# ychalier/transflow

Hardware: AMD Instinct MI355X
Metric: frames/sec (Farneback+remap) (higher is better)
Workload: dtype f32; 1 GPU; 4k: one clip of T=256 3840x2160 uint8 frames sharded over the ranks (rank r owns pairs shard_range(255, r, 1) + a one-frame halo), Farneback pyr_scale=0.5 levels=5 winsize=15 iterations=3 poly_n=5 poly_sigma=1.2 flags=0, BACKWARD post_process, moveref layer (reset random p=0.5 through a float mask, u drawn on the GPU), 1 RGB pixmap source, render; clip_frames=256, equal_batches=False

## Files before the change

### transflow_amd/csrc/common.h

```cpp
#pragma once
#include <hip/hip_runtime.h>

#include <cstdarg>
#include <cstdint>
#include <cstdio>
#include <cstdlib>
#include <memory>
#include <new>
#include <string>
#include <vector>

#include "../../include/tfhip.h"

#define TF_API extern "C" __attribute__((visibility("default")))

namespace tf {

int set_error(int code, const char *fmt, ...) __attribute__((format(printf, 2, 3)));
hipStream_t stream();
hipStream_t main_stream();
int side_stream(int which, hipStream_t *out);
int ensure_init();

enum Opt { OPT_FB_FUSED = 0, OPT_FB_FUSE_MIN_PX, OPT_FB_NO_SHARE, OPT_FB_NO_OVERLAP, OPT_REMAP_PX, OPT_REMAP_NO_PACK, OPT_REMAP_KEEP_RGBA,
           OPT_PROF_LEVELS, OPT_FB_EXACT_SUMS, OPT_FB_CHAIN, OPT_FB_SEGS, OPT_REMAP_QUAD, OPT_JD_PAR_SUB_BYTES,
           OPT_JD_PAR_GROUP_SUBS, OPT_JD_PAR_STAGED, OPT_REMAP_LEAN, OPT_COUNT };
long option(Opt which);

#ifdef TF_EXPERIMENT
inline long tune(const char *env, long dflt)
{
    const char *v = getenv(env);
    return v ? atol(v) : dflt;
}
inline const char *tune_str(const char *env) { return getenv(env); }
#else
constexpr long tune(const char *, long dflt) { return dflt; }
constexpr const char *tune_str(const char *) { return nullptr; }
#endif

struct StreamScope {
    explicit StreamScope(hipStream_t s);
    ~StreamScope();
    hipStream_t prev;
};

#define TF_HIP(expr)                                                                              \
    do {                                                                                          \
        hipError_t _e = (expr);                                                                   \
        if (_e != hipSuccess)                                                                     \
            return tf::set_error(TF_ERR_HIP, "%s failed: %s (%s:%d)", #expr, hipGetErrorString(_e), \
                                 __FILE__, __LINE__);                                             \
    } while (0)

#define TF_TRY(expr)        \
    do {                    \
        int _rc = (expr);   \
        if (_rc != TF_OK)   \
            return _rc;     \
// ... 110 lines not shown
```

### transflow_amd/csrc/fb_common.h

```cpp
#pragma once
#include <type_traits>
#include <algorithm>
#include <cfloat>
#include <cmath>
#include <cstdlib>
#include <cstring>
#include <map>
#include <memory>
#include <mutex>
#include <string>

#include "common.h"
#include "fb_plan.h"

struct tf_fb;

namespace tf {
namespace fb {

constexpr int MAX_POLY_N = 15;

typedef float float2u __attribute__((ext_vector_type(2), aligned(4)));
typedef float float4u __attribute__((ext_vector_type(4), aligned(4)));

// ... 86 lines not shown
    const unsigned u = (xcd < rn ? xcd * (qn + 1) : rn * (qn + 1) + (xcd - rn) * qn) + (lin >> 3);
    const unsigned whole = u / (S * G);
    unsigned l = 0;
    while (l < 7 && (l + 1) * P / 8 <= whole)
        l++;
    const unsigned p0 = l * P / 8, n = (l + 1) * P / 8 - p0, r = u - p0 * S * G;
    by = r / (S * n);
    const unsigned rem = r - by * S * n;
    bx = rem / n;
    pair = (int)(p0 + (rem - bx * n));
}

__device__ __forceinline__ void lds_barrier()
{
    __builtin_amdgcn_fence(__ATOMIC_RELEASE, "workgroup", "local");
    __builtin_amdgcn_s_barrier();
    __builtin_amdgcn_fence(__ATOMIC_ACQUIRE, "workgroup", "local");
}
__device__ __forceinline__ double fast_recip(double d)
{
    const double r = __builtin_amdgcn_rcp(d);
    return __builtin_fma(__builtin_fma(-d, r, 1.0), r, r);
}

__device__ __forceinline__ void lds_wave_sync()
{
    __builtin_amdgcn_fence(__ATOMIC_RELEASE, "workgroup", "local");
    __builtin_amdgcn_wave_barrier();
    __builtin_amdgcn_fence(__ATOMIC_ACQUIRE, "workgroup", "local");
}

__device__ __forceinline__ int reflect101_once(int p, int len) { return p < 0 ? -p : (p >= len ? 2 * len - 2 - p : p); }
__device__ __forceinline__ int reflect101_near(int p, int len) { return len < 2 ? 0 : reflect101_once(p, len); }

struct ImgTile {
    int TWo, THo;
    int tw_shift;
    int rstride;
    int LW, LH;
    int pitch;
    int same_size;
    double scale_x, scale_y;
};

typedef float f32x2 __attribute__((ext_vector_type(2)));
typedef float f32x4 __attribute__((ext_vector_type(4)));

constexpr int RP_MAX_LEVELS = 4;

__device__ __forceinline__ float border_weight(int d) { return d < 2 ? 0.14f : (d < 5 ? 0.4472f : 1.f); }
__device__ __forceinline__ float border_scale(int x, int y, int W, int H)
{
    const bool fires = (unsigned)(x - 5) >= (unsigned)(W - 10) || (unsigned)(y - 5) >= (unsigned)(H - 10);
    return fires ? border_weight(x) * border_weight(W - x - 1) * border_weight(y) * border_weight(H - y - 1) : 1.f;
}

struct FlowInit {
    int mode;
    const float2 *src;
    int Wc, Hc;
    const int *xofs, *yofs;
    const float *xfrac, *yfrac;
    float mul;
    const int2 *rmap;
};

// ... 113 lines not shown
namespace fb {

inline FlowInit fb_upsampled(tf_fb *fb, int k, const float2 *coarse_flow)
{
    const Level &L = *fb->lv[k], &C = *fb->lv[k + 1];
    FlowInit fi;
    memset(&fi, 0, sizeof(fi));
    fi.mode = 1;
    fi.src = coarse_flow;
    fi.Wc = C.W;
    fi.Hc = C.H;
    fi.xofs = L.flow_lerp.xofs.as<int>();
    fi.yofs = L.flow_lerp.yofs.as<int>();
    fi.xfrac = L.flow_lerp.xfrac.as<float>();
    fi.yfrac = L.flow_lerp.yfrac.as<float>();
    fi.mul = (float)(1. / fb->prm.pyr_scale);
    return fi;
}

inline bool fb_exact(const tf_fb *fb) { return fb->exact >= 0 ? fb->exact != 0 : option(OPT_FB_EXACT_SUMS) != 0; }

struct March {
    int mode, segs, seg;
};

const char *lvl_name(const char *base, int k);

int fb_level_image(tf_fb *fb, int k, const ImageRun &run, bool standalone = false);
bool plan_split_level(int W, int H, Level &L, std::vector<int> &colsrc);
bool plan_quarter_level(int W, int H, const Level &L);
ImgTile choose_tile(int W, int H, int Wk, int Hk, int ksz, int level);
int fb_polyexp(tf_fb *fb, int w, int h, const ImageRun &run, int k = -1);
int fb_expand_level(tf_fb *fb, int k, const ImageRun &run, bool standalone = false);
int fb_m_room(tf_fb *fb, int w, int h, int n_pairs);
int fb_update_matrices(tf_fb *fb, int w, int h, int n_pairs, const FlowInit &fi, int k = -1);
int fb_carry_room(tf_fb *fb, size_t carry_doubles, size_t flags);
int fb_check_fault(tf_fb *fb, const char *where);
int fb_carry_scan(tf_fb *fb, int w, int n_pairs, int segs, int k);
int fb_blur_solve(tf_fb *fb, int w, int h, int n_pairs, float2 *flow_out, int k = -1);
int fb_gauss_solve(tf_fb *fb, int w, int h, int n_pairs, float2 *flow_out, int k = -1);
int fb_setup_flags(tf_fb *fb);
int fb_initial_flow(tf_fb *fb, int n_pairs, float2 *out);
int fb_exact_room(tf_fb *fb, int w, int h, int n_pairs);
int fb_exact_from_matrices(tf_fb *fb, int w, int h, int n_pairs, float2 *flow_out, int k);
int fb_exact_hsolve(tf_fb *fb, int w, int h, int n_pairs, float2 *flow_out, int k);
int fb_w1_solve(tf_fb *fb, int w, int h, int n_pairs, float2 *flow_out);
bool fb_flow_iter_serves(const tf_fb *fb, int w, int h);
int fb_flow_iter(tf_fb *fb, int w, int h, int n_pairs, float2 *flow_out, int k, const FlowInit &fi);

}
}
```

### transflow_amd/csrc/fb_level_image.hip

```cpp
#include "fb_common.h"

namespace {

__device__ __forceinline__ int lerp_coord(int d, double scale, int src, bool zero_at_edges, float &frac)
{
    float f = (float)((d + 0.5) * scale - 0.5);
    int s = (int)floorf(f);
    f -= s;
    if (zero_at_edges) {
        if (s < 0) {
            f = 0.f;
            s = 0;
        }
        if (s >= src - 1) {
            f = 0.f;
            s = src - 1;
        }
    }
    frac = f;
    return s;
}

__global__ void __launch_bounds__(256)
k_level_image(const uint8_t *__restrict__ frames, const int2 *__restrict__ pairs, float *__restrict__ img, int W,
// ... 345 lines not shown
            float *out = L.rowf + (out_row0 + row) * NC + 4 * grp;
            out[0] = acc0.x;
            out[1] = acc1.x;
            if (four) {
                out[2] = acc0.y;
                out[3] = acc1.y;
            }
        }
    }
}

__global__ void __launch_bounds__(RP_THREADS)
k_level_rowpass(const uint8_t *__restrict__ frames, const int2 *__restrict__ pairs, int W, int H, RowPassArgs args, int RB,
                int pitch, int r4, int rmax)
{
    extern __shared__ __attribute__((aligned(16))) uint8_t s_rp[];
    uint8_t *sS = s_rp;
    float *sKall = reinterpret_cast<float *>(s_rp + (size_t)RB * pitch);
    const int pi = blockIdx.y;
    const int2 pr = pairs[pi >> 1];
    const uint8_t *src = frames + (size_t)((pi & 1) ? pr.y : pr.x) * W * H;
    const int y0 = blockIdx.x * RB, nrows = min(RB, H - y0);
    {
        int base = 0;
        for (int l = 0; l < args.n; l++) {
            for (int i = threadIdx.x; i < args.lv[l].ksz; i += RP_THREADS)
                sKall[base + i] = args.lv[l].kern[i];
            base += args.lv[l].ksz;
        }
    }
    const int nq = W >> 2;
    {
        const int lane_ = threadIdx.x & 63, wave_ = threadIdx.x >> 6;
        constexpr int U = 4;
        for (int i = wave_; i < nrows; i += RP_WAVES) {
            const uint32_t *g = reinterpret_cast<const uint32_t *>(src + (size_t)(y0 + i) * W);
            uint32_t *d = reinterpret_cast<uint32_t *>(sS + i * pitch + r4);
            for (int c0 = lane_; c0 < nq; c0 += 64 * U) {
                uint32_t v[U];
#pragma unroll
                for (int u = 0; u < U; u++)
                    if (c0 + 64 * u < nq)
                        v[u] = g[c0 + 64 * u];
#pragma unroll
                for (int u = 0; u < U; u++)
                    if (c0 + 64 * u < nq)
                        d[c0 + 64 * u] = v[u];
            }
        }
    }
    for (int idx = threadIdx.x; idx < nrows * 2 * rmax; idx += RP_THREADS) {
        const int i = idx / (2 * rmax), j = idx - i * 2 * rmax;
        const int c = j < rmax ? j - rmax : W + (j - rmax);
        sS[i * pitch + r4 + c] = src[(size_t)(y0 + i) * W + reflect101(c, W)];
    }
    __syncthreads();
    const int lane = threadIdx.x & 63, wave = threadIdx.x >> 6;
    int kbase = 0;
    for (int l = 0; l < args.n; l++) {
        const RowPassLevel &L = args.lv[l];
        const float *sK = sKall + kbase;
        kbase += L.ksz;
        const size_t out_row0 = (size_t)pi * H + y0;
        if (L.ksz == 9 && L.rshift == 1) {
            rowpass_level_t<9, 1>(L, sS, sK, nrows, pitch, r4, out_row0, lane, wave);
            continue;
        }
        if (L.ksz == 19 && L.rshift == 2) {
            rowpass_level_t<19, 2>(L, sS, sK, nrows, pitch, r4, out_row0, lane, wave);
            continue;
        }
        if (L.ksz == 39 && L.rshift == 3) {
            rowpass_level_t<39, 3>(L, sS, sK, nrows, pitch, r4, out_row0, lane, wave);
            continue;
        }
        if (L.ksz == 79 && L.rshift == 3) {
            rowpass_level_t<79, 3>(L, sS, sK, nrows, pitch, r4, out_row0, lane, wave);
            continue;
        }
        const int ksz = L.ksz, r = ksz >> 1, NC = L.NC, rshift = L.rshift;
        const int R = 1 << rshift, G = 64 >> rshift;
        const int li = lane & (R - 1), lg = lane >> rshift;
        const int ngroups = (NC + 3) >> 2;
        const int n_rb = (nrows + R - 1) >> rshift, n_gb = (ngroups + G - 1) / G;
        for (int item = wave; item < n_rb * n_gb; item += RP_WAVES) {
            const int gb = item % n_gb, rb = item / n_gb;
            const int row = rb * R + li, grp = gb * G + lg;
// ... 161 lines not shown
    const int Wk = W >> 2, Hk = H >> 2;
    unsigned tbx, tby, tbz;
    xcd_tile3(tbx, tby, tbz);
    const int pi = tbz;
    const int2 pr = pairs[pi >> 1];
    const uint8_t *src = frames + (size_t)((pi & 1) ? pr.y : pr.x) * W * H;
    const int X0 = tbx * QI_TW, Y0 = tby * QI_TH;
    const int lane = threadIdx.x & 63, wave = threadIdx.x >> 6;
    const int xs = S * X0 - 4, ys = S * Y0 - 3;
    const bool dwords = xs >= 0 && xs + 4 * PD <= W && ys >= 0 && ys + NR <= H;
    if (dwords) {
        constexpr int U = (NR + 3) / 4;
        for (int j0 = wave; j0 < NR; j0 += 4 * U) {
            uint32_t v[U], v2[U];
#pragma unroll
            for (int u = 0; u < U; u++) {
                const int j = min(j0 + 4 * u, NR - 1);
                const uint32_t *g = reinterpret_cast<const uint32_t *>(src + (size_t)(ys + j) * W + xs);
                v[u] = g[lane];
                v2[u] = g[64 + (lane & 1)];
            }
#pragma unroll
            for (int u = 0; u < U; u++) {
                const int j = j0 + 4 * u;
                if (j < NR) {
                    sS[j * PD + lane] = v[u];
                    if (lane < 2)
                        sS[j * PD + 64 + lane] = v2[u];
                }
            }
        }
    } else {
        uint8_t *s8 = reinterpret_cast<uint8_t *>(sS);
        for (int j = wave; j < NR; j += 4) {
            const uint8_t *g = src + (size_t)reflect101(ys + j, H) * W;
            for (int b = lane; b < 4 * PD; b += 64)
                s8[j * 4 * PD + b] = g[reflect101(xs + b, W)];
        }
    }
    __syncthreads();
    const int X = X0 + lane, Yw = Y0 + SEG * wave;
    if (X >= Wk || Yw >= Hk)
        return;
    float t[K];
#pragma unroll
    for (int i = 0; i < K; i++)
        t[i] = kern[i];
    const float fx = xfrac[X];
    const uint32_t *q = sS + (S * SEG * wave) * PD + lane;
    constexpr int NROWS = S * (SEG - 1) + 2 + 2 * r;
    float c0[NROWS], c1[NROWS];
    auto row_pair = [&](int j) {
        const uint32_t *qa = q + j * PD, *qb = qa + PD;
        const uint32_t a0 = qa[0], a1 = qa[1], a2 = qa[2], b0 = qb[0], b1 = qb[1], b2 = qb[2];
        const uint32_t wa[3] = {__builtin_amdgcn_alignbyte(a1, a0, 1), __builtin_amdgcn_alignbyte(a2, a1, 1), a2 >> 8};
        const uint32_t wb[3] = {__builtin_amdgcn_alignbyte(b1, b0, 1), __builtin_amdgcn_alignbyte(b2, b1, 1), b2 >> 8};
        f32x2 p[K + 1];
#pragma unroll
        for (int i = 0; i <= K; i++)
            p[i] = f32x2{(float)((wa[i >> 2] >> (8 * (i & 3))) & 0xff), (float)((wb[i >> 2] >> (8 * (i & 3))) & 0xff)};
        f32x2 A0 = t[0] * p[0], A1 = t[0] * p[1];
#pragma unroll
        for (int i = 1; i < K; i++) {
            A0 += t[i] * p[i];
            A1 += t[i] * p[i + 1];
        }
        c0[j] = A0.x;
        c0[j + 1] = A0.y;
        c1[j] = A1.x;
        c1[j + 1] = A1.y;
    };
#pragma unroll
    for (int j = 0; j < 6; j += 2)
        row_pair(j);
    float *dst = img + (size_t)pi * Wk * Hk + X;
#pragma unroll
    for (int y = 0; y < SEG; y++) {
        if (Yw + y >= Hk)
            break;
        row_pair(S * y + 6);
        row_pair(S * y + 8);
        const int m = S * y + r;
        float v00 = t[r] * c0[m], v01 = t[r] * c1[m], v10 = t[r] * c0[m + 1], v11 = t[r] * c1[m + 1];
#pragma unroll
        for (int i = 1; i <= r; i++) {
            const float k = t[r + i];
            v00 += k * (c0[m + i] + c0[m - i]);
            v01 += k * (c1[m + i] + c1[m - i]);
            v10 += k * (c0[m + 1 + i] + c0[m + 1 - i]);
            v11 += k * (c1[m + 1 + i] + c1[m + 1 - i]);
        }
        const float fy = yfrac[Yw + y];
        const float h0 = v00 * (1.f - fx) + v01 * fx, h1 = v10 * (1.f - fx) + v11 * fx;
        dst[(size_t)(Yw + y) * Wk] = h0 * (1.f - fy) + h1 * fy;
    }
}

}

namespace tf {
namespace fb {

int fb_level_image(tf_fb *fb, int k, const ImageRun &run, bool standalone)
{
    Level &L = *fb->lv[k];
    if (L.quarter)
        return launch(lvl_name("fb_level_image", k), k_level_quarter_image, dim3(cdiv(L.W, QI_TW), cdiv(L.H, QI_TH), run.n),
                      dim3(256), 0, (const uint8_t *)fb->frames.as<uint8_t>(), fb->image_list(run), fb->imgk(k), fb->W, fb->H,
                      (const float *)L.kern.as<float>(), (const float *)L.img_lerp.xfrac.as<float>(),
                      (const float *)L.img_lerp.yfrac.as<float>());
    if (L.split) {
        if (k == fb->rp_first || standalone) {
            RowPassArgs a;
            memset(&a, 0, sizeof(a));
            size_t taps = 0;
            for (int j = fb->K; j >= 1; j--) {
                Level &S = *fb->lv[j];
                if (!S.split)
                    continue;
                RowPassLevel &rl = a.lv[a.n++];
                rl.rowf = fb->rowf.as<float>() + S.rowf_off;
                rl.colsrc = S.colsrc.as<int>();
                rl.kern = S.kern.as<float>();
                rl.NC = S.NC;
                rl.ksz = S.ksz;
                rl.rshift = S.rp_rshift;
                taps += (size_t)S.ksz;
            }
            const size_t smem_rp = (size_t)fb->rp_RB * fb->rp_pitch + taps * sizeof(float);
            TF_TRY(launch(lvl_name("fb_level_rowpass", -1), k_level_rowpass, dim3(cdiv(fb->H, fb->rp_RB), run.n),
                          dim3(RP_THREADS), smem_rp, (const uint8_t *)fb->frames.as<uint8_t>(),
                          fb->image_list(run), fb->W, fb->H, a, fb->rp_RB, fb->rp_pitch, fb->rp_r4,
                          fb->rp_rmax));
        }
        return launch(lvl_name("fb_level_colpass", k), k_level_colpass, dim3(cdiv(L.W, 64), cdiv(L.H, 4), run.n), dim3(256),
                      (size_t)L.ksz * sizeof(float), (const float *)(fb->rowf.as<float>() + L.rowf_off), fb->imgk(k), fb->W, fb->H,
                      L.W, L.H, L.NC, (const float *)L.kern.as<float>(), L.ksz, (const int *)L.img_lerp.xofs.as<int>(),
                      (const float *)L.img_lerp.xfrac.as<float>(), (const int *)L.img_lerp.yofs.as<int>(),
// ... 139 lines not shown
```

### transflow_amd/csrc/fb_pyramid.hip

```cpp
#include "fb_common.h"

namespace {

#ifndef TF_PX_TH
#define TF_PX_TH 16
#endif
constexpr int PX_TW = 64, PX_TH = TF_PX_TH;

__global__ void k_polyexp(const float *__restrict__ img, float *__restrict__ R, int Wk, int Hk, PolyConst pc)
{
    extern __shared__ float s_mem[];
    const int n = pc.n;
    const int LW = PX_TW + 2 * n;
    const int LH = PX_TH + 2 * n;
    float *sI = s_mem;
    float *sT = s_mem + LH * LW;
    const int pi = blockIdx.z;
    const size_t Nk = (size_t)Wk * Hk;
    const float *src = img + (size_t)pi * Nk;
    const int x0 = blockIdx.x * PX_TW, y0 = blockIdx.y * PX_TH;
    for (int idx = threadIdx.x; idx < LH * LW; idx += blockDim.x) {
        int ry = idx / LW, cx = idx % LW;
        int y = clampi(y0 - n + ry, 0, Hk - 1), x = clampi(x0 - n + cx, 0, Wk - 1);
        sI[idx] = src[(size_t)y * Wk + x];
// ... 48 lines not shown
        r_store_px(dst, Nk, o, v);
    }
}

typedef float float2w __attribute__((ext_vector_type(2), aligned(4)));

template <int N>
__device__ __forceinline__ void polyexp_vertical4(const f32x2 (&v)[4 + 2 * N], const PolyConst &pc, float *T0, float *T1,
                                                  float *T2, int LW)
{
#pragma unroll
    for (int q = 0; q < 4; q++) {
        const f32x2 c = v[q + N];
        f32x2 t0 = c * pc.g[0], t1 = {0.f, 0.f}, t2 = {0.f, 0.f};
#pragma unroll
        for (int k = 1; k <= N; k++) {
            const f32x2 a = v[q + N - k], b = v[q + N + k];
            const f32x2 p = a + b;
            t0 = t0 + pc.g[k] * p;
            t1 = t1 + pc.xg[k] * (b - a);
            t2 = t2 + pc.xxg[k] * p;
        }
        *reinterpret_cast<f32x2 *>(T0 + q * LW) = t0;
        *reinterpret_cast<f32x2 *>(T1 + q * LW) = t1;
        *reinterpret_cast<f32x2 *>(T2 + q * LW) = t2;
    }
}

template <int N>
__global__ void __launch_bounds__(256)
k_polyexp_t(const float *__restrict__ img, float *__restrict__ R, int Wk, int Hk, PolyConst pc)
{
    constexpr int TW = PX_TW, TH = PX_TH, LW = TW + 2 * N, LH = TH + 2 * N;
    __shared__ float sI[LH * LW];
    __shared__ float sT[3][TH][LW];
    const int pi = blockIdx.z;
    const size_t Nk = (size_t)Wk * Hk;
    const float *src = img + (size_t)pi * Nk;
    const int x0 = blockIdx.x * TW, y0 = blockIdx.y * TH;
    for (int idx = threadIdx.x; idx < LH * LW; idx += 256) {
        int ry = idx / LW, cx = idx - ry * LW;
        int y = clampi(y0 - N + ry, 0, Hk - 1), x = clampi(x0 - N + cx, 0, Wk - 1);
        sI[idx] = src[(size_t)y * Wk + x];
    }
    __syncthreads();
    static_assert(LW % 2 == 0, "column pairs");
    for (int idx = threadIdx.x; idx < (TH / 4) * (LW / 2); idx += 256) {
        const int g = idx / (LW / 2), cx = 2 * (idx - g * (LW / 2));
        f32x2 v[4 + 2 * N];
#pragma unroll
        for (int j = 0; j < 4 + 2 * N; j++)
            v[j] = *reinterpret_cast<const f32x2 *>(&sI[(4 * g + j) * LW + cx]);
        polyexp_vertical4<N>(v, pc, &sT[0][4 * g][cx], &sT[1][4 * g][cx], &sT[2][4 * g][cx], LW);
    }
    __syncthreads();
    float *dst = R + (size_t)pi * 5 * Nk;
    for (int idx = threadIdx.x; idx < TH * (TW / 2); idx += 256) {
        const int ty = idx / (TW / 2), cp = idx - ty * (TW / 2);
        const int x = x0 + 2 * cp, y = y0 + ty;
        if (x >= Wk || y >= Hk)
            continue;
        float w0[2 + 2 * N], w1[2 + 2 * N], w2[2 + 2 * N];
#pragma unroll
        for (int j = 0; j < 2 + 2 * N; j++) {
            w0[j] = sT[0][ty][2 * cp + j];
            w1[j] = sT[1][ty][2 * cp + j];
            w2[j] = sT[2][ty][2 * cp + j];
        }
        float out[2][5];
#pragma unroll
        for (int q = 0; q < 2; q++) {
            const float *T0 = w0 + q + N, *T1 = w1 + q + N, *T2 = w2 + q + N;
            float g0 = pc.g[0];
            double b1 = T0[0] * g0, b2 = 0, b3 = T1[0] * g0, b4 = 0, b5 = T2[0] * g0, b6 = 0;
#pragma unroll
            for (int k = 1; k <= N; k++) {
// ... 236 lines not shown
                        *reinterpret_cast<uint32_t *>(sS + ry * SW + 4 * c) = v[u];
                }
            }
        }
    } else {
        for (int c = lane; c < ncols; c += 64) {
            const int x = reflect101_near(xs + c, W);
            for (int j0 = wave; j0 < nrows; j0 += 4 * U) {
                uint8_t v[U];
#pragma unroll
                for (int u = 0; u < U; u++) {
                    int ry = j0 + 4 * u;
                    if (ry < nrows)
                        v[u] = src[(size_t)reflect101_near(rfirst + ry, H) * W + x];
                }
#pragma unroll
                for (int u = 0; u < U; u++) {
                    int ry = j0 + 4 * u;
                    if (ry < nrows)
                        sS[ry * SW + c] = v[u];
                }
            }
        }
    }
    __syncthreads();
    static_assert(LW % 2 == 0 && SW >= 2 * LW + 8, "2 x 2 blocks; a block's three dwords stay inside its staged row");
    for (int idx = threadIdx.x; idx < ((ny + 1) >> 1) * (LW / 2); idx += 256) {
        const int by2 = idx / (LW / 2), ry = 2 * by2, cx = 2 * (idx - by2 * (LW / 2));
        float rp[6][4];
#pragma unroll
        for (int dy = 0; dy < 6; dy++) {
            const uint32_t *q = reinterpret_cast<const uint32_t *>(sS + (2 * ry + dy) * SW + 2 * cx);
            const uint32_t d0 = q[0], d1 = q[1], d2 = q[2];
            const uint32_t lo = __builtin_amdgcn_alignbyte(d1, d0, off), hi = __builtin_amdgcn_alignbyte(d2, d1, off);
            const float b0 = (float)(lo & 0xff), b1 = (float)((lo >> 8) & 0xff), b2 = (float)((lo >> 16) & 0xff),
                        b3 = (float)(lo >> 24), b4 = (float)(hi & 0xff), b5 = (float)((hi >> 8) & 0xff);
            rp[dy][0] = b1 * kc + (b0 + b2) * k1;
            rp[dy][1] = b2 * kc + (b1 + b3) * k1;
            rp[dy][2] = b3 * kc + (b2 + b4) * k1;
            rp[dy][3] = b4 * kc + (b3 + b5) * k1;
        }
#pragma unroll
        for (int a = 0; a < 2; a++) {
            float out[2];
#pragma unroll
            for (int b = 0; b < 2; b++) {
                float v00 = kc * rp[2 * a + 1][2 * b], v01 = kc * rp[2 * a + 1][2 * b + 1];
                float v10 = kc * rp[2 * a + 2][2 * b], v11 = kc * rp[2 * a + 2][2 * b + 1];
                v00 += k1 * (rp[2 * a + 2][2 * b] + rp[2 * a][2 * b]);
                v01 += k1 * (rp[2 * a + 2][2 * b + 1] + rp[2 * a][2 * b + 1]);
                v10 += k1 * (rp[2 * a + 3][2 * b] + rp[2 * a + 1][2 * b]);
                v11 += k1 * (rp[2 * a + 3][2 * b + 1] + rp[2 * a + 1][2 * b + 1]);
                const float h0 = v00 * (1.f - 0.5f) + v01 * 0.5f, h1 = v10 * (1.f - 0.5f) + v11 * 0.5f;
                out[b] = h0 * (1.f - 0.5f) + h1 * 0.5f;
            }
            if (ry + a < ny)
                *reinterpret_cast<f32x2 *>(sI + (ry + a) * LW + cx) = f32x2{out[0], out[1]};
        }
    }
    __syncthreads();
    tile_expansion<N, TW, TH>(sI, sT, x0, y0, xr0, yr0, Wk, Hk, pc, R + (size_t)pi * 5 * Nk, Nk);
}

}

namespace tf {
namespace fb {

int fb_polyexp(tf_fb *fb, int w, int h, const ImageRun &run, int k)
{
    const int n = fb->pc.n;
    dim3 grid(cdiv(w, PX_TW), cdiv(h, PX_TH), run.n);
    if (n == 5)
        return launch(lvl_name("fb_polyexp", k), k_polyexp_t<5>, grid, dim3(256), 0, (const float *)fb->imgk(k),
                      fb->Rk(k, run), w, h, fb->pc);
    if (n == 7)
        return launch(lvl_name("fb_polyexp", k), k_polyexp_t<7>, grid, dim3(256), 0, (const float *)fb->imgk(k),
                      fb->Rk(k, run), w, h, fb->pc);
    size_t smem = ((size_t)(PX_TH + 2 * n) * (PX_TW + 2 * n) + 3 * (size_t)PX_TH * (PX_TW + 2 * n)) * sizeof(float);
    return launch(lvl_name("fb_polyexp_generic", k), k_polyexp, grid, dim3(256), smem,
                  (const float *)fb->imgk(k), fb->Rk(k, run), w, h, fb->pc);
}

static bool fb_can_fuse_level(tf_fb *fb, int k)
{
    static const bool off = tune("TF_FB_NO_A1A2", 0) != 0;
    const Level &L = *fb->lv[k];
    return !off && L.W == fb->W && L.H == fb->H && L.ksz == 3 && (fb->pc.n == 5 || fb->pc.n == 7);
}

static bool fb_can_fuse_half_level(tf_fb *fb, int k)
{
    static const bool off = tune("TF_FB_NO_A1A2", 0) != 0;
    const Level &L = *fb->lv[k];
    return !off && 2 * L.W == fb->W && 2 * L.H == fb->H && L.ksz == 3 && (fb->pc.n == 5 || fb->pc.n == 7);
}

static int fb_level1_polyexp(tf_fb *fb, int k, const ImageRun &run)
{
    Level &L = *fb->lv[k];
    dim3 grid(cdiv(L.W, 64), cdiv(L.H, TF_EXP_TH1), run.n);
    const float kc = L.kern_host[1], k1 = L.kern_host[2];
    if (fb->pc.n == 5)
        return launch(lvl_name("fb_level_polyexp", k), k_level1_polyexp_t<5>, grid, dim3(256), 0,
                      (const uint8_t *)fb->frames.as<uint8_t>(), fb->image_list(run), fb->Rk(k, run), fb->W,
                      fb->H, kc, k1, fb->pc);
    return launch(lvl_name("fb_level_polyexp", k), k_level1_polyexp_t<7>, grid, dim3(256), 0,
                  (const uint8_t *)fb->frames.as<uint8_t>(), fb->image_list(run), fb->Rk(k, run), fb->W, fb->H,
                  kc, k1, fb->pc);
}

static int fb_level0_polyexp(tf_fb *fb, int k, const ImageRun &run)
{
    Level &L = *fb->lv[k];
    dim3 grid(cdiv(L.W, 64), cdiv(L.H, TF_EXP_TH0), run.n);
    const float kc = L.kern_host[1], k1 = L.kern_host[2];
    if (fb->pc.n == 5)
        return launch(lvl_name("fb_level_polyexp", k), k_level0_polyexp_t<5>, grid, dim3(256), 0,
                      (const uint8_t *)fb->frames.as<uint8_t>(), fb->image_list(run), fb->Rk(k, run),
                      L.W, L.H, kc, k1, fb->pc);
    return launch(lvl_name("fb_level_polyexp", k), k_level0_polyexp_t<7>, grid, dim3(256), 0,
                  (const uint8_t *)fb->frames.as<uint8_t>(), fb->image_list(run), fb->Rk(k, run), L.W,
                  L.H, kc, k1, fb->pc);
}

int fb_expand_level(tf_fb *fb, int k, const ImageRun &run, bool standalone)
{
    if (fb_can_fuse_level(fb, k))
        return fb_level0_polyexp(fb, k, run);
    if (fb_can_fuse_half_level(fb, k))
        return fb_level1_polyexp(fb, k, run);
    TF_TRY(fb_level_image(fb, k, run, standalone));
    return fb_polyexp(fb, fb->lv[k]->W, fb->lv[k]->H, run, k);
}

}
}
```

### transflow_amd/csrc/runtime.hip

```cpp
#include <cstring>
#include <map>
#include <mutex>

#include "common.h"

#include <cstdlib>

namespace tf {

static thread_local std::string g_last_error;
static std::mutex g_mu;
static bool g_inited = false;
static int g_device = 0;
static hipStream_t g_stream = nullptr;

int set_error(int code, const char *fmt, ...)
{
    char buf[1024];
    va_list ap;
    va_start(ap, fmt);
    vsnprintf(buf, sizeof(buf), fmt, ap);
    va_end(ap);
    g_last_error = buf;
    return code;
}

struct OptDef {
    const char *name;
    long value, lo, hi;
};
static OptDef g_opts[OPT_COUNT] = {
    {"fb_fused", -1, -1, 1},
    {"fb_fuse_min_px", 4000000, 0, 1l << 40},
    {"fb_no_share", 0, 0, 1},
    {"fb_no_overlap", 0, 0, 1},
    {"remap_px", 4, 1, 4},
    {"remap_no_pack", 0, 0, 2},
    {"remap_keep_rgba", 0, 0, 1},
    {"prof_levels", 0, 0, 1},
    {"fb_exact_sums", 0, 0, 1},
    {"fb_chain", -1, -1, 1},
    {"fb_segs", 0, 0, 64},
    {"remap_quad", 1, 0, 1},
    {"jd_par_sub_bytes", 0, 0, 1024},
    {"jd_par_group_subs", 0, 0, 256},
    {"jd_par_staged", 0, 0, 1},
    {"remap_lean", 1, 0, 1},
};
long option(Opt which) { return g_opts[which].value; }

static thread_local hipStream_t g_override = nullptr;
static thread_local hipStream_t g_thread_main = nullptr;
static hipStream_t g_thread_streams[3] = {nullptr, nullptr, nullptr};

hipStream_t main_stream() { return g_thread_main ? g_thread_main : g_stream; }
hipStream_t stream() { return g_override ? g_override : main_stream(); }

static hipStream_t g_side[5] = {nullptr, nullptr, nullptr, nullptr, nullptr};
int side_stream(int which, hipStream_t *out)
{
    TF_REQUIRE(which >= 0 && which <= 4, "side_stream: bad index");
    TF_TRY(ensure_init());
    std::lock_guard<std::mutex> lk(g_mu);
    if (!g_side[which]) {
        int least = 0, greatest = 0;
        TF_HIP(hipDeviceGetStreamPriorityRange(&least, &greatest));
        TF_HIP(hipStreamCreateWithPriority(&g_side[which], hipStreamNonBlocking, (which == 0 || which >= 3) ? least : greatest));
    }
    *out = g_side[which];
    return TF_OK;
}

StreamScope::StreamScope(hipStream_t s) : prev(g_override) { g_override = s; }
StreamScope::~StreamScope() { g_override = prev; }

static int init_device(int device)
{
    std::lock_guard<std::mutex> lk(g_mu);
    if (g_inited) {
        if (device != g_device)
// ... 446 lines not shown
```

### transflow_amd/roofline.py

```python
from __future__ import annotations

import json
import os

HBM_PEAK_GBS = 8000.0
HBM_COPY_CEILING_GBS = 6290.0

_ROOT = os.path.dirname(os.path.dirname(os.path.abspath(__file__)))


def level_sizes(width: int, height: int, pyr_scale: float, levels: int):
    k, scale = 0, 1.0
    while k < levels:
        scale *= pyr_scale
        if width * scale < 32 or height * scale < 32:
            break
        k += 1
    out = []
    for lvl in range(k + 1):
        s = 1.0
        for _ in range(lvl):
            s *= pyr_scale
        out.append((int(round_half_even(width * s)), int(round_half_even(height * s))))
    return out
# ... 59 lines not shown
            continue
        if name == "fb_level_polyexp" and k >= 2:
            continue
        if name == "fb_polyexp" and k < 2:
            continue
        if name == "fb_flow_iter" and not level_is_fused(n[k], pairs, fused):
            continue
        if name in ("fb_update_matrices", "fb_blur_solve") and level_is_fused(n[k], pairs, fused):
            continue
        if name == "fb_blur_solve":
            mult = iterations
        elif name in ("fb_update_matrices", "fb_flow_iter"):
            total += (iterations - 1) * pairs * (68 if name == "fb_update_matrices" else 96) * n[k]
        total += mult * kernel_bytes(name, n[0], n[k], nc, pairs)
    return total


def built_kernel_bytes(name, width, height, levels, pairs, iterations=3, fused=-1) -> int:
    n, sizes = _levels(width, height, levels)
    frames = pairs + 1
    total = 0
    if name.startswith("remap_step"):
        return 0
    for k in range(len(n)):
        nc = n[k + 1] if k + 1 < len(n) else 0
        is_fused = level_is_fused(n[k], pairs, fused)
        if name == "fb_flow_iter" and is_fused:
            first = 48 * n[k] + (8 * nc if nc else 0)
            total += pairs * (first + (iterations - 1) * 56 * n[k])
        elif name == "fb_update_matrices" and not is_fused:
            total += pairs * (60 * n[k] + (8 * nc if nc else 0) + (iterations - 1) * 68 * n[k])
        elif name == "fb_blur_solve" and not is_fused:
            total += pairs * iterations * 28 * n[k]
        elif name == "fb_level_polyexp" and k < 2:
            total += frames * (n[0] + 20 * n[k])
        elif name == "fb_level_rowpass" and k >= 2:
            if k == 2:
                total += frames * n[0]
            total += frames * 8 * sizes[0][1] * sizes[k][0]
        elif name == "fb_level_colpass" and k >= 2:
            total += frames * (8 * sizes[0][1] * sizes[k][0] + 4 * n[k])
        elif name == "fb_polyexp" and k >= 2:
            total += frames * 24 * n[k]
    return total


def built_flow_iter_level_bytes(width, height, levels, pairs, iterations=3, fused=-1) -> dict:
    n, _ = _levels(width, height, levels)
    out = {}
    for k in range(len(n)):
        nc = n[k + 1] if k + 1 < len(n) else 0
        if level_is_fused(n[k], pairs, fused):
            out[k] = pairs * (48 * n[k] + (8 * nc if nc else 0) + (iterations - 1) * 56 * n[k])
    return out


BUILT_FB_KERNELS = ("fb_flow_iter", "fb_update_matrices", "fb_blur_solve", "fb_level_polyexp", "fb_level_rowpass",
                    "fb_level_colpass", "fb_polyexp")


def built_remap_bytes(width, height, reset_mask=False, forward=False) -> int:
    state = 8 if width <= 8192 and height <= 8192 else 16
    per_px = (4 + 16 if forward else 8) + state + 3 + 4 + 3 + (4 if reset_mask else 0)
    return per_px * width * height


def built_step_bytes(width, height, levels, pairs, iterations=3, reset_mask=False, forward=False, fused=-1) -> int:
    fb = sum(built_kernel_bytes(k, width, height, levels, pairs, iterations, fused) for k in BUILT_FB_KERNELS)
    rm = pairs * built_remap_bytes(width, height, reset_mask, forward)
    if not forward and pairs >= 2:
        rm -= (pairs - 1) * 4 * width * height
    return fb + rm


def profile_traffic(name, width, height, levels, pairs, launches_per_step, iterations=3, fused=-1):
    table = None
    for fname in ("r05_traffic.json", "r04_traffic.json", "r03_traffic.json", "r02_traffic.json", "r01_traffic.json"):
        path = os.path.join(_ROOT, "profiles", fname)
        if os.path.exists(path):
            with open(path) as f:
                t = json.load(f)
            if name in t:
                table = t
                break
    if table is None:
        return None
    n, _ = _levels(width, height, levels)
    per_level_launches = {"fb_update_matrices": iterations, "fb_blur_solve": iterations,
                          "fb_flow_iter": iterations}.get(name, 1)
    if name == "fb_flow_iter":
        n = [v for v in n if level_is_fused(v, pairs, fused)]
# ... 24 lines not shown
```

Before: 2138 frames/s.

## Split fused level-1 polyexp into standalone half-image kernel plus generic polyexp

Adds a default-on option that splits pyramid level 1 out of the fused downsample+polynomial-expansion kernel. A new register-walking half-resolution image kernel reads the uint8 frame directly and writes a float image, and the generic polyexp then runs on that image. Separately, it batches the global-to-LDS staging loads in the row-pass, quarter-image and polyexp tile kernels (more loads in flight, vectorised float2 loads for interior tiles). Splitting adds an intermediate float image round trip through memory, in exchange for dropping the fused kernel's redundant halo recomputation and LDS pressure.

```diff
diff --git a/transflow_amd/csrc/common.h b/transflow_amd/csrc/common.h
--- a/transflow_amd/csrc/common.h
+++ b/transflow_amd/csrc/common.h
@@ -24,7 +24,7 @@
 
 enum Opt { OPT_FB_FUSED = 0, OPT_FB_FUSE_MIN_PX, OPT_FB_NO_SHARE, OPT_FB_NO_OVERLAP, OPT_REMAP_PX, OPT_REMAP_NO_PACK, OPT_REMAP_KEEP_RGBA,
            OPT_PROF_LEVELS, OPT_FB_EXACT_SUMS, OPT_FB_CHAIN, OPT_FB_SEGS, OPT_REMAP_QUAD, OPT_JD_PAR_SUB_BYTES,
-           OPT_JD_PAR_GROUP_SUBS, OPT_JD_PAR_STAGED, OPT_REMAP_LEAN, OPT_COUNT };
+           OPT_JD_PAR_GROUP_SUBS, OPT_JD_PAR_STAGED, OPT_REMAP_LEAN, OPT_FB_LEVEL1_SPLIT, OPT_COUNT };
 long option(Opt which);
 
 #ifdef TF_EXPERIMENT
diff --git a/transflow_amd/csrc/fb_common.h b/transflow_amd/csrc/fb_common.h
--- a/transflow_amd/csrc/fb_common.h
+++ b/transflow_amd/csrc/fb_common.h
@@ -142,6 +142,33 @@
 
 __device__ __forceinline__ int reflect101_once(int p, int len) { return p < 0 ? -p : (p >= len ? 2 * len - 2 - p : p); }
 __device__ __forceinline__ int reflect101_near(int p, int len) { return len < 2 ? 0 : reflect101_once(p, len); }
+
+__device__ __forceinline__ void half_level_row_pass(uint32_t lo, uint32_t hi, float kc, float k1, float rp[4])
+{
+    const float b0 = (float)(lo & 0xff), b1 = (float)((lo >> 8) & 0xff), b2 = (float)((lo >> 16) & 0xff),
+                b3 = (float)(lo >> 24), b4 = (float)(hi & 0xff), b5 = (float)((hi >> 8) & 0xff);
+    rp[0] = b1 * kc + (b0 + b2) * k1;
+    rp[1] = b2 * kc + (b1 + b3) * k1;
+    rp[2] = b3 * kc + (b2 + b4) * k1;
+    rp[3] = b4 * kc + (b3 + b5) * k1;
+}
+__device__ __forceinline__ void half_level_block(const float (&rp)[6][4], float kc, float k1, float out[2][2])
+{
+#pragma unroll
+    for (int a = 0; a < 2; a++) {
+#pragma unroll
+        for (int b = 0; b < 2; b++) {
+            float v00 = kc * rp[2 * a + 1][2 * b], v01 = kc * rp[2 * a + 1][2 * b + 1];
+            float v10 = kc * rp[2 * a + 2][2 * b], v11 = kc * rp[2 * a + 2][2 * b + 1];
+            v00 += k1 * (rp[2 * a + 2][2 * b] + rp[2 * a][2 * b]);
+            v01 += k1 * (rp[2 * a + 2][2 * b + 1] + rp[2 * a][2 * b + 1]);
+            v10 += k1 * (rp[2 * a + 3][2 * b] + rp[2 * a + 1][2 * b]);
+            v11 += k1 * (rp[2 * a + 3][2 * b + 1] + rp[2 * a + 1][2 * b + 1]);
+            const float h0 = v00 * (1.f - 0.5f) + v01 * 0.5f, h1 = v10 * (1.f - 0.5f) + v11 * 0.5f;
+            out[a][b] = h0 * (1.f - 0.5f) + h1 * 0.5f;
+        }
+    }
+}
 
 struct ImgTile {
     int TWo, THo;
@@ -321,6 +348,7 @@
 ImgTile choose_tile(int W, int H, int Wk, int Hk, int ksz, int level);
 int fb_polyexp(tf_fb *fb, int w, int h, const ImageRun &run, int k = -1);
 int fb_expand_level(tf_fb *fb, int k, const ImageRun &run, bool standalone = false);
+bool fb_split_half_level(tf_fb *fb, int k);
 int fb_m_room(tf_fb *fb, int w, int h, int n_pairs);
 int fb_update_matrices(tf_fb *fb, int w, int h, int n_pairs, const FlowInit &fi, int k = -1);
 int fb_carry_room(tf_fb *fb, size_t carry_doubles, size_t flags);
diff --git a/transflow_amd/csrc/fb_level_image.hip b/transflow_amd/csrc/fb_level_image.hip
--- a/transflow_amd/csrc/fb_level_image.hip
+++ b/transflow_amd/csrc/fb_level_image.hip
@@ -401,27 +401,53 @@
     const int nq = W >> 2;
     {
         const int lane_ = threadIdx.x & 63, wave_ = threadIdx.x >> 6;
-        constexpr int U = 4;
-        for (int i = wave_; i < nrows; i += RP_WAVES) {
+        constexpr int U = 16;
+        for (int i = wave_; i < nrows; i += 2 * RP_WAVES) {
+            const int i2 = i + RP_WAVES;
+            const bool second = i2 < nrows;
             const uint32_t *g = reinterpret_cast<const uint32_t *>(src + (size_t)(y0 + i) * W);
+            const uint32_t *g2 = reinterpret_cast<const uint32_t *>(src + (size_t)(y0 + (second ? i2 : i)) * W);
             uint32_t *d = reinterpret_cast<uint32_t *>(sS + i * pitch + r4);
+            uint32_t *d2 = reinterpret_cast<uint32_t *>(sS + i2 * pitch + r4);
             for (int c0 = lane_; c0 < nq; c0 += 64 * U) {
-                uint32_t v[U];
+                uint32_t v[U], v2[U];
 #pragma unroll
                 for (int u = 0; u < U; u++)
-                    if (c0 + 64 * u < nq)
+                    if (c0 + 64 * u < nq) {
                         v[u] = g[c0 + 64 * u];
+                        v2[u] = g2[c0 + 64 * u];
+                    }
 #pragma unroll
                 for (int u = 0; u < U; u++)
-                    if (c0 + 64 * u < nq)
+                    if (c0 + 64 * u < nq) {
                         d[c0 + 64 * u] = v[u];
-            }
-        }
-    }
-    for (int idx = threadIdx.x; idx < nrows * 2 * rmax; idx += RP_THREADS) {
-        const int i = idx / (2 * rmax), j = idx - i * 2 * rmax;
-        const int c = j < rmax ? j - rmax : W + (j - rmax);
-        sS[i * pitch + r4 + c] = src[(size_t)(y0 + i) * W + reflect101(c, W)];
+                        if (second)
+                            d2[c0 + 64 * u] = v2[u];
+                    }
+            }
+        }
+    }
+    {
+        constexpr int UH = 4;
+        const int nh = nrows * 2 * rmax;
+        for (int idx0 = threadIdx.x; idx0 < nh; idx0 += RP_THREADS * UH) {
+            uint8_t v[UH];
+            int at[UH];
+#pragma unroll
+            for (int u = 0; u < UH; u++) {
+                const int idx = idx0 + RP_THREADS * u;
+                if (idx < nh) {
+                    const int i = idx / (2 * rmax), j = idx - i * 2 * rmax;
+                    const int c = j < rmax ? j - rmax : W + (j - rmax);
+                    at[u] = i * pitch + r4 + c;
+                    v[u] = src[(size_t)(y0 + i) * W + reflect101(c, W)];
+                }
+            }
+#pragma unroll
+            for (int u = 0; u < UH; u++)
+                if (idx0 + RP_THREADS * u < nh)
+                    sS[at[u]] = v[u];
+        }
     }
     __syncthreads();
     const int lane = threadIdx.x & 63, wave = threadIdx.x >> 6;
@@ -649,10 +675,28 @@
         }
     } else {
         uint8_t *s8 = reinterpret_cast<uint8_t *>(sS);
-        for (int j = wave; j < NR; j += 4) {
-            const uint8_t *g = src + (size_t)reflect101(ys + j, H) * W;
-            for (int b = lane; b < 4 * PD; b += 64)
-                s8[j * 4 * PD + b] = g[reflect101(xs + b, W)];
+        constexpr int CB = (4 * PD + 63) / 64, RU = 4;
+        int col[CB];
+#pragma unroll
+        for (int u = 0; u < CB; u++)
+            col[u] = reflect101(xs + min(lane + 64 * u, 4 * PD - 1), W);
+        for (int j0 = wave; j0 < NR; j0 += 4 * RU) {
+            uint8_t v[RU][CB];
+#pragma unroll
+            for (int q = 0; q < RU; q++) {
+                const uint8_t *g = src + (size_t)reflect101(ys + min(j0 + 4 * q, NR - 1), H) * W;
+#pragma unroll
+                for (int u = 0; u < CB; u++)
+                    v[q][u] = g[col[u]];
+            }
+#pragma unroll
+            for (int q = 0; q < RU; q++) {
+                const int j = j0 + 4 * q;
+#pragma unroll
+                for (int u = 0; u < CB; u++)
+                    if (j < NR && lane + 64 * u < 4 * PD)
+                        s8[j * 4 * PD + lane + 64 * u] = v[q][u];
+            }
         }
     }
     __syncthreads();
@@ -713,6 +757,107 @@
     }
 }
 
+constexpr int HI_BLOCKS = 4;
+
+template <bool DWORDS>
+__device__ __forceinline__ void half_image_walk(const uint8_t *__restrict__ src, float *__restrict__ dst, int W, int H, int Wk, int Hk,
+                                                int X, int Y0, float kc, float k1)
+{
+    constexpr int NV = DWORDS ? 3 : 6;
+    const bool left = X == 0, right = 2 * X + 4 >= W;
+    int col[6];
+#pragma unroll
+    for (int dx = 0; dx < 6; dx++)
+        col[dx] = reflect101_near(min(2 * X - 1 + dx, W), W);
+    auto fetch = [&](int fr, uint32_t(&v)[NV]) {
+        const uint8_t *g = src + (size_t)reflect101_near(min(fr, H), H) * W;
+        if constexpr (DWORDS) {
+            const uint32_t *q = reinterpret_cast<const uint32_t *>(g + 2 * X);
+            v[1] = q[0];
+            v[0] = left ? 0u : q[-1];
+            v[2] = right ? 0u : q[1];
+        } else {
+#pragma unroll
+            for (int dx = 0; dx < NV; dx++)
+                v[dx] = g[col[dx]];
+        }
+    };
+    auto row_pass = [&](const uint32_t(&v)[NV], float rp[4]) {
+        uint32_t lo, hi;
+        if constexpr (DWORDS) {
+            const uint32_t a = left ? v[1] << 16 : v[0], c = right ? v[1] >> 16 : v[2];
+            lo = __builtin_amdgcn_alignbyte(v[1], a, 3);
+            hi = __builtin_amdgcn_alignbyte(c, v[1], 3);
+        } else {
+            lo = v[0] | v[1] << 8 | v[2] << 16 | v[3] << 24;
+            hi = v[4] | v[5] << 8;
+        }
+        half_level_row_pass(lo, hi, kc, k1, rp);
+    };
+    uint32_t first[2][NV], next[4][NV];
+    fetch(2 * Y0 - 1, first[0]);
+    fetch(2 * Y0, first[1]);
+#pragma unroll
+    for (int q = 0; q < 4; q++)
+        fetch(2 * Y0 + 1 + q, next[q]);
+    float rp[6][4];
+    row_pass(first[0], rp[0]);
+    row_pass(first[1], rp[1]);
+#pragma unroll
+    for (int blk = 0; blk < HI_BLOCKS; blk++) {
+        const int Y = Y0 + 2 * blk;
+        if (Y >= Hk)
+            break;
+        uint32_t cur[4][NV];
+#pragma unroll
+        for (int q = 0; q < 4; q++)
+#pragma unroll
+            for (int j = 0; j < NV; j++)
+                cur[q][j] = next[q][j];
+        if (blk + 1 < HI_BLOCKS) {
+#pragma unroll
+            for (int q = 0; q < 4; q++)
+                fetch(2 * Y + 5 + q, next[q]);
+        }
+#pragma unroll
+        for (int q = 0; q < 4; q++)
+            row_pass(cur[q], rp[2 + q]);
+        float out[2][2];
+        half_level_block(rp, kc, k1, out);
+        float *o = dst + (size_t)Y * Wk + X;
+#pragma unroll
+        for (int a = 0; a < 2; a++) {
+            if (Y + a < Hk) {
+                if (X + 1 < Wk)
+                    *reinterpret_cast<float2u *>(o + (size_t)a * Wk) = float2u{out[a][0], out[a][1]};
+                else
+                    o[(size_t)a * Wk] = out[a][0];
+            }
+        }
+#pragma unroll
+        for (int j = 0; j < 4; j++) {
+            rp[0][j] = rp[4][j];
+            rp[1][j] = rp[5][j];
+        }
+    }
+}
+
+template <bool DWORDS>
+__global__ void __launch_bounds__(256)
+k_level_half_image(const uint8_t *__restrict__ frames, const int2 *__restrict__ pairs, float *__restrict__ img, int W, int H,
+                   float kc, float k1)
+{
+    const int Wk = W >> 1, Hk = H >> 1;
+    const int pi = blockIdx.z;
+    const int2 pr = pairs[pi >> 1];
+    const uint8_t *src = frames + (size_t)((pi & 1) ? pr.y : pr.x) * W * H;
+    const int X = 2 * (blockIdx.x * 64 + (threadIdx.x & 63)), Y0 = 2 * HI_BLOCKS * (blockIdx.y * 4 + (threadIdx.x >> 6));
+    if (X >= Wk || Y0 >= Hk)
+        return;
+    float *dst = img + (size_t)pi * Wk * Hk;
+    half_image_walk<DWORDS>(src, dst, W, H, Wk, Hk, X, Y0, kc, k1);
+}
+
 }
 
 namespace tf {
@@ -721,6 +866,11 @@
 int fb_level_image(tf_fb *fb, int k, const ImageRun &run, bool standalone)
 {
     Level &L = *fb->lv[k];
+    if (fb_split_half_level(fb, k))
+        return launch(lvl_name("fb_level_image", k), (fb->W & 3) == 0 ? k_level_half_image<true> : k_level_half_image<false>,
+                      dim3(cdiv(L.W, 128), cdiv(L.H, 8 * HI_BLOCKS), run.n), dim3(256), 0,
+                      (const uint8_t *)fb->frames.as<uint8_t>(), fb->image_list(run), fb->imgk(k), fb->W, fb->H,
+                      L.kern_host[1], L.kern_host[2]);
     if (L.quarter)
         return launch(lvl_name("fb_level_image", k), k_level_quarter_image, dim3(cdiv(L.W, QI_TW), cdiv(L.H, QI_TH), run.n),
                       dim3(256), 0, (const uint8_t *)fb->frames.as<uint8_t>(), fb->image_list(run), fb->imgk(k), fb->W, fb->H,
diff --git a/transflow_amd/csrc/fb_pyramid.hip b/transflow_amd/csrc/fb_pyramid.hip
--- a/transflow_amd/csrc/fb_pyramid.hip
+++ b/transflow_amd/csrc/fb_pyramid.hip
@@ -104,16 +104,49 @@
 k_polyexp_t(const float *__restrict__ img, float *__restrict__ R, int Wk, int Hk, PolyConst pc)
 {
     constexpr int TW = PX_TW, TH = PX_TH, LW = TW + 2 * N, LH = TH + 2 * N;
-    __shared__ float sI[LH * LW];
+    __shared__ __attribute__((aligned(8))) float sI[LH * LW];
     __shared__ float sT[3][TH][LW];
     const int pi = blockIdx.z;
     const size_t Nk = (size_t)Wk * Hk;
     const float *src = img + (size_t)pi * Nk;
     const int x0 = blockIdx.x * TW, y0 = blockIdx.y * TH;
-    for (int idx = threadIdx.x; idx < LH * LW; idx += 256) {
-        int ry = idx / LW, cx = idx - ry * LW;
-        int y = clampi(y0 - N + ry, 0, Hk - 1), x = clampi(x0 - N + cx, 0, Wk - 1);
-        sI[idx] = src[(size_t)y * Wk + x];
+    static_assert(LW % 2 == 0, "column pairs");
+    if (x0 - N >= 0 && x0 + TW - 1 + N <= Wk - 1 && y0 - N >= 0 && y0 + TH - 1 + N <= Hk - 1) {
+        constexpr int PW = LW / 2, NP = (LH * PW + 255) / 256, DR = 256 / PW, DC = 256 % PW;
+        const float *base = src + (size_t)(y0 - N) * Wk + (x0 - N);
+        const int ry = threadIdx.x / PW;
+        int cp = threadIdx.x - ry * PW, o = ry * Wk + 2 * cp;
+        float2u v[NP];
+#pragma unroll
+        for (int u = 0; u < NP; u++) {
+            if ((u + 1) * 256 <= LH * PW || threadIdx.x + u * 256 < LH * PW)
+                v[u] = *reinterpret_cast<const float2u *>(base + o);
+            const bool wrap = cp + DC >= PW;
+            cp += wrap ? DC - PW : DC;
+            o += DR * Wk + 2 * DC + (wrap ? Wk - LW : 0);
+        }
+#pragma unroll
+        for (int u = 0; u < NP; u++)
+            if ((u + 1) * 256 <= LH * PW || threadIdx.x + u * 256 < LH * PW)
+                *reinterpret_cast<f32x2 *>(&sI[2 * (threadIdx.x + u * 256)]) = f32x2{v[u].x, v[u].y};
+    } else {
+        constexpr int NS = (LH * LW + 255) / 256, DR = 256 / LW, DC = 256 % LW;
+        int ry = threadIdx.x / LW, cx = threadIdx.x - ry * LW;
+        float v[NS];
+#pragma unroll
+        for (int u = 0; u < NS; u++) {
+            if ((u + 1) * 256 <= LH * LW || threadIdx.x + u * 256 < LH * LW) {
+                const int y = clampi(y0 - N + ry, 0, Hk - 1), x = clampi(x0 - N + cx, 0, Wk - 1);
+                v[u] = src[(size_t)y * Wk + x];
+            }
+            const bool wrap = cx + DC >= LW;
+            cx += wrap ? DC - LW : DC;
+            ry += wrap ? DR + 1 : DR;
+        }
+#pragma unroll
+        for (int u = 0; u < NS; u++)
+            if ((u + 1) * 256 <= LH * LW || threadIdx.x + u * 256 < LH * LW)
+                sI[threadIdx.x + u * 256] = v[u];
     }
     __syncthreads();
     static_assert(LW % 2 == 0, "column pairs");
@@ -416,31 +449,14 @@
         for (int dy = 0; dy < 6; dy++) {
             const uint32_t *q = reinterpret_cast<const uint32_t *>(sS + (2 * ry + dy) * SW + 2 * cx);
             const uint32_t d0 = q[0], d1 = q[1], d2 = q[2];
-            const uint32_t lo = __builtin_amdgcn_alignbyte(d1, d0, off), hi = __builtin_amdgcn_alignbyte(d2, d1, off);
-            const float b0 = (float)(lo & 0xff), b1 = (float)((lo >> 8) & 0xff), b2 = (float)((lo >> 16) & 0xff),
-                        b3 = (float)(lo >> 24), b4 = (float)(hi & 0xff), b5 = (float)((hi >> 8) & 0xff);
-            rp[dy][0] = b1 * kc + (b0 + b2) * k1;
-            rp[dy][1] = b2 * kc + (b1 + b3) * k1;
-            rp[dy][2] = b3 * kc + (b2 + b4) * k1;
-            rp[dy][3] = b4 * kc + (b3 + b5) * k1;
-        }
-#pragma unroll
-        for (int a = 0; a < 2; a++) {
-            float out[2];
-#pragma unroll
-            for (int b = 0; b < 2; b++) {
-                float v00 = kc * rp[2 * a + 1][2 * b], v01 = kc * rp[2 * a + 1][2 * b + 1];
-                float v10 = kc * rp[2 * a + 2][2 * b], v11 = kc * rp[2 * a + 2][2 * b + 1];
-                v00 += k1 * (rp[2 * a + 2][2 * b] + rp[2 * a][2 * b]);
-                v01 += k1 * (rp[2 * a + 2][2 * b + 1] + rp[2 * a][2 * b + 1]);
-                v10 += k1 * (rp[2 * a + 3][2 * b] + rp[2 * a + 1][2 * b]);
-                v11 += k1 * (rp[2 * a + 3][2 * b + 1] + rp[2 * a + 1][2 * b + 1]);
-                const float h0 = v00 * (1.f - 0.5f) + v01 * 0.5f, h1 = v10 * (1.f - 0.5f) + v11 * 0.5f;
-                out[b] = h0 * (1.f - 0.5f) + h1 * 0.5f;
-            }
+            half_level_row_pass(__builtin_amdgcn_alignbyte(d1, d0, off), __builtin_amdgcn_alignbyte(d2, d1, off), kc, k1, rp[dy]);
+        }
+        float out[2][2];
+        half_level_block(rp, kc, k1, out);
+#pragma unroll
+        for (int a = 0; a < 2; a++)
             if (ry + a < ny)
-                *reinterpret_cast<f32x2 *>(sI + (ry + a) * LW + cx) = f32x2{out[0], out[1]};
-        }
+                *reinterpret_cast<f32x2 *>(sI + (ry + a) * LW + cx) = f32x2{out[a][0], out[a][1]};
     }
     __syncthreads();
     tile_expansion<N, TW, TH>(sI, sT, x0, y0, xr0, yr0, Wk, Hk, pc, R + (size_t)pi * 5 * Nk, Nk);
@@ -480,6 +496,8 @@
     return !off && 2 * L.W == fb->W && 2 * L.H == fb->H && L.ksz == 3 && (fb->pc.n == 5 || fb->pc.n == 7);
 }
 
+bool fb_split_half_level(tf_fb *fb, int k) { return k >= 1 && fb_can_fuse_half_level(fb, k) && option(OPT_FB_LEVEL1_SPLIT) != 0; }
+
 static int fb_level1_polyexp(tf_fb *fb, int k, const ImageRun &run)
 {
     Level &L = *fb->lv[k];
@@ -512,7 +530,7 @@
 {
     if (fb_can_fuse_level(fb, k))
         return fb_level0_polyexp(fb, k, run);
-    if (fb_can_fuse_half_level(fb, k))
+    if (fb_can_fuse_half_level(fb, k) && !fb_split_half_level(fb, k))
         return fb_level1_polyexp(fb, k, run);
     TF_TRY(fb_level_image(fb, k, run, standalone));
     return fb_polyexp(fb, fb->lv[k]->W, fb->lv[k]->H, run, k);
diff --git a/transflow_amd/csrc/runtime.hip b/transflow_amd/csrc/runtime.hip
--- a/transflow_amd/csrc/runtime.hip
+++ b/transflow_amd/csrc/runtime.hip
@@ -46,6 +46,7 @@
     {"jd_par_group_subs", 0, 0, 256},
     {"jd_par_staged", 0, 0, 1},
     {"remap_lean", 1, 0, 1},
+    {"fb_level1_split", 1, 0, 1},
 };
 long option(Opt which) { return g_opts[which].value; }
 
diff --git a/transflow_amd/roofline.py b/transflow_amd/roofline.py
--- a/transflow_amd/roofline.py
+++ b/transflow_amd/roofline.py
@@ -115,8 +115,12 @@
             total += pairs * (60 * n[k] + (8 * nc if nc else 0) + (iterations - 1) * 68 * n[k])
         elif name == "fb_blur_solve" and not is_fused:
             total += pairs * iterations * 28 * n[k]
-        elif name == "fb_level_polyexp" and k < 2:
+        elif name == "fb_level_polyexp" and k < 1:
             total += frames * (n[0] + 20 * n[k])
+        elif name == "fb_level_image" and k == 1:
+            total += frames * (n[0] + 4 * n[k])
+        elif name == "fb_polyexp" and k == 1:
+            total += frames * 24 * n[k]
         elif name == "fb_level_rowpass" and k >= 2:
             if k == 2:
                 total += frames * n[0]
@@ -138,8 +142,8 @@
     return out
 
 
-BUILT_FB_KERNELS = ("fb_flow_iter", "fb_update_matrices", "fb_blur_solve", "fb_level_polyexp", "fb_level_rowpass",
-                    "fb_level_colpass", "fb_polyexp")
+BUILT_FB_KERNELS = ("fb_flow_iter", "fb_update_matrices", "fb_blur_solve", "fb_level_polyexp", "fb_level_image",
+                    "fb_level_rowpass", "fb_level_colpass", "fb_polyexp")
 
 
 def built_remap_bytes(width, height, reset_mask=False, forward=False) -> int:
```

Result: no change. 2129 frames/s (-0.4%).
